# A-Nasiri-M/sap3d_tensorflow

Hardware: AMD Instinct MI355X
Metric: clips/s (16x112x112 fwd+bwd) (higher is better)
Workload: dtype f32

## Files before the change

### include/p3d_hip.h

```cpp
#ifndef P3D_HIP_H
#define P3D_HIP_H
#include <stddef.h>
#include <stdint.h>

#ifdef __cplusplus
extern "C" {
#endif

typedef struct p3d_handle p3d_handle;

enum {
    P3D_STRUCTURE_UNET = 0,
    P3D_STRUCTURE_CONCAT = 1,
    P3D_STRUCTURE_GN_P3D = 2,
    P3D_STRUCTURE_UNETPP_NONSA = 3,
    P3D_STRUCTURE_GN_P3D_DECODER = 4,
    P3D_STRUCTURE_GN_P3D_CONCAT = 5,
    P3D_STRUCTURE_UNETPP_DS = 6
};

typedef struct p3d_config {
    int structure;
    int batch;
    int frames;
// ... 134 lines not shown
                   float b2, float eps, int lr_on_device, float* lr_t);
int p3d_debug_optimizer(int device, int kind, float* p, float* g, float* m, int64_t n, int offset, float lr, float momentum,
                        int use_nesterov, int lr_on_device);
int p3d_debug_optimizer_decay(int device, int kind, float* p, float* g, float* m, int64_t n, int offset, const int64_t* tile_off,
                              const int64_t* tile_len, const float* tile_c, int ntile, float lr, float momentum, int use_nesterov,
                              int lr_on_device, int update, double* term);
int p3d_debug_stat_parts(const int64_t xshape[5], const int64_t wshape[5], const int s[3], int transpose, int* written, int* cap);
int p3d_debug_igemm_groupable(const int64_t xshape[5], const int64_t wshape[5], const int s[3]);
int p3d_op_max_pool3d(int device, const float* x, const int64_t xshape[5], const int ksize[3], const int s[3], float* y);
int p3d_op_max_pool3d_grad(int device, const float* x, const int64_t xshape[5], const int ksize[3], const int s[3],
                           const float* dy, float* dx);
int p3d_op_bias_add_grad(int device, const float* dy, int64_t rows, int channels, float* dbias);
int p3d_debug_conv_launch(int device, int kind, const float* in, int ld_in, int off_in, const int64_t xshape[5], const float* w,
                          const int64_t wshape[5], const int s[3], const float* bias, int accum, int f16, float* out, int ld_out,
                          int off_out, char* kernels, int kernels_cap, int* splits);
int p3d_debug_wgrad_group(int device, int n, const float* const* x, const int* ldx, const int* offx, const int64_t* xs,
                          const float* const* dy, const int* lddy, const int* offdy, const int64_t* ws, const int* s, const int* transpose,
                          float* const* dw, float* const* dbias, int polite, int greedy, char* kernel, int kernel_cap, int* cuts,
                          int* info);
int p3d_debug_max_pool3d(int device, const float* x, int ldx, int offx, const int64_t xshape[5], const int ksize[3], const int s[3],
                         float* y, int ldy, int offy);
int p3d_debug_max_pool3d_grad(int device, const float* x, int ldx, int offx, const int64_t xshape[5], const int ksize[3], const int s[3],
                              const float* dy, int ldy, int offy, int accumulate, float* dx, const char** kernel);
int p3d_debug_bias_add_grad(int device, const float* dy, int64_t rows, int channels, int ld, int off, float* dbias);
int p3d_op_attention_core(int device, int batch, int n_g, int n_f, int ch, const float* g, const float* f, const float* h,
                          float* o, const float* d_o, float* dg, float* df, float* dh);
int p3d_debug_attention_core(int device, int mode, int batch, int n_g, int n_f, int ch, const float* g, const float* f, const float* h,
                             float* o, const float* d_o, float* dg, float* df, float* dh);
int p3d_debug_attention_splits(int batch, int n_g, int n_f, int ch, int splits[4]);
int p3d_debug_softmax_rows(int device, int backward, int64_t rows, int cols, int ld, float* s, float* d, int guard_rows);
// ... 32 lines not shown
```

### sap3d_tensorflow_amd/_lib.py

```python
import ctypes as C
import os

_HERE = os.path.dirname(os.path.abspath(__file__))
LIB_PATH = os.environ.get("P3D_LIB") or os.path.join(_HERE, "libp3dhip.so")

P3D_COMM_ID_BYTES = 128
LOSSES = {"smooth_l1": 0, "bce": 1, "l1": 2}
P3D_LOSS_KLD_CC = 3
MAP_LOSSES = {"kld": (1.0, 0.0), "kld_cc": (1.0, 1.0)}
REGULARIZATION = {"weightdecay": 1, "l2": 2}
OPTIMIZERS = {"adam": 0, "momentum": 1, "sgd": 2}
SLOT_NAMES = {"adam": ("Adam", "Adam_1"), "momentum": ("Momentum",), "sgd": ()}


class P3dConfig(C.Structure):
    _fields_ = [("structure", C.c_int), ("batch", C.c_int), ("frames", C.c_int), ("height", C.c_int),
                ("width", C.c_int), ("base", C.c_int), ("blocks", C.c_int * 3), ("device", C.c_int),
                ("world_size", C.c_int), ("rank", C.c_int)]


class P3dOpTime(C.Structure):
    _fields_ = [("name", C.c_char * 64), ("kernel", C.c_char * 48), ("ms", C.c_double), ("flops", C.c_double),
                ("bytes", C.c_double), ("phase", C.c_int)]

# ... 83 lines not shown
    "p3d_debug_optimizer": (C.c_int, [C.c_int, C.c_int, _fp, _fp, _fp, C.c_int64, C.c_int, C.c_float, C.c_float, C.c_int, C.c_int]),
    "p3d_debug_optimizer_decay": (C.c_int, [C.c_int, C.c_int, _fp, _fp, _fp, C.c_int64, C.c_int, _i64p, _i64p, _fp, C.c_int, C.c_float,
                                            C.c_float, C.c_int, C.c_int, C.c_int, _dp]),
    "p3d_debug_adam": (C.c_int, [C.c_int, _fp, _fp, _fp, _fp, C.c_int64, C.c_int, C.c_float, C.c_int64, C.c_float, C.c_float,
                                 C.c_float, C.c_int, _fp]),
    "p3d_debug_stat_parts": (C.c_int, [_i64p, _i64p, _ip, C.c_int, _ip, _ip]),
    "p3d_debug_igemm_groupable": (C.c_int, [_i64p, _i64p, _ip]),
    "p3d_op_conv3d_backprop_input": (C.c_int, [C.c_int, _fp, _fp, _i64p, _ip, _i64p, _fp]),
    "p3d_op_conv3d_backprop_filter": (C.c_int, [C.c_int, _fp, _i64p, _fp, _i64p, _ip, _fp, _fp]),
    "p3d_op_conv3d_transpose": (C.c_int, [C.c_int, _fp, _i64p, _fp, _i64p, _ip, _fp, _fp]),
    "p3d_op_max_pool3d": (C.c_int, [C.c_int, _fp, _i64p, _ip, _ip, _fp]),
    "p3d_op_max_pool3d_grad": (C.c_int, [C.c_int, _fp, _i64p, _ip, _ip, _fp, _fp]),
    "p3d_op_bias_add_grad": (C.c_int, [C.c_int, _fp, C.c_int64, C.c_int, _fp]),
    "p3d_debug_conv_launch": (C.c_int, [C.c_int, C.c_int, _fp, C.c_int, C.c_int, _i64p, _fp, _i64p, _ip, _fp, C.c_int, C.c_int, _fp,
                                        C.c_int, C.c_int, C.c_char_p, C.c_int, _ip]),
    "p3d_debug_wgrad_group": (C.c_int, [C.c_int, C.c_int, C.POINTER(_fp), _ip, _ip, _i64p, C.POINTER(_fp), _ip, _ip, _i64p, _ip, _ip,
                                        C.POINTER(_fp), C.POINTER(_fp), C.c_int, C.c_int, C.c_char_p, C.c_int, _ip, _ip]),
    "p3d_debug_max_pool3d": (C.c_int, [C.c_int, _fp, C.c_int, C.c_int, _i64p, _ip, _ip, _fp, C.c_int, C.c_int]),
    "p3d_debug_max_pool3d_grad": (C.c_int, [C.c_int, _fp, C.c_int, C.c_int, _i64p, _ip, _ip, _fp, C.c_int, C.c_int, C.c_int, _fp,
                                            C.POINTER(C.c_char_p)]),
    "p3d_debug_bias_add_grad": (C.c_int, [C.c_int, _fp, C.c_int64, C.c_int, C.c_int, C.c_int, _fp]),
    "p3d_op_attention_core": (C.c_int, [C.c_int, C.c_int, C.c_int, C.c_int, C.c_int, _fp, _fp, _fp, _fp, _fp, _fp, _fp, _fp]),
    "p3d_debug_attention_core": (C.c_int, [C.c_int, C.c_int, C.c_int, C.c_int, C.c_int, C.c_int, _fp, _fp, _fp, _fp, _fp, _fp, _fp, _fp]),
    "p3d_debug_attention_splits": (C.c_int, [C.c_int, C.c_int, C.c_int, C.c_int, _ip]),
    "p3d_debug_softmax_rows": (C.c_int, [C.c_int, C.c_int, C.c_int64, C.c_int, C.c_int, _fp, _fp, C.c_int]),
    "p3d_debug_attn_mix": (C.c_int, [C.c_int, C.c_int64, C.c_int, _fp, C.c_int, C.c_int, _fp, C.c_int, C.c_int, C.c_float, C.c_float,
                                     C.c_uint64, C.c_int, _fp, C.c_int, C.c_int, _fp, C.c_int, _fp, _fp, _fp]),
    "p3d_metric_cc": (C.c_int, [C.c_int, _fp, _fp, C.c_int, C.c_int, _dp]),
    "p3d_metric_sim": (C.c_int, [C.c_int, _fp, _fp, C.c_int, C.c_int, _dp]),
    "p3d_metric_nss": (C.c_int, [C.c_int, _fp, _fp, C.c_int, C.c_int, _dp]),
# ... 116 lines not shown
```

### sap3d_tensorflow_amd/csrc/conv_igemm2.hip

```cpp
#if !defined(__gfx950__) && !defined(__gfx942__) && defined(__HIP_DEVICE_COMPILE__)
#error "the K-slice exchange (write-through slab stores + relaxed ticket + one-lane acquire) is written for gfx942 / gfx950 cache semantics"
#endif
#include "p3d_kernels.h"
#include "igemm_epilogue.h"
#include <algorithm>
#include <cstddef>
#include <cstdio>
#include <cstring>
#include <cstdlib>
#include <map>
#include <mutex>
#include <tuple>
#include <vector>

typedef float f32x16 __attribute__((ext_vector_type(16)));
typedef unsigned u32x4 __attribute__((ext_vector_type(4)));

namespace {

constexpr int BK = 32;
#ifndef P3D_RING64
#define P3D_RING64 3
#endif
template <int BM, int BN>
// ... 72 lines not shown
    } else {
#pragma unroll
        for (int i = 0; i < LB; ++i) {
            const int r = (i * 4 + wave) * 8 + a_sub;
            st.bk[i] = 4 * (a_slot ^ ((r >> 1) & 7));
            st.bok[i] = (n0 + r) < p.Nc;
            st.boff[i] = (n0 + r) * p.K + st.bk[i];
        }
    }
    st.t = s_begin / kchunks; st.kc = s_begin - st.t * kchunks; st.issued = 0;
}

template <int LA, bool TWO>
__device__ __forceinline__ void a_set_tap(const IgemmArgs& p, P3dKTap* taps, ALoad<LA, TWO>& st) {
    const P3dTap tap = p3d_ktap(taps, st.t);
#pragma unroll
    for (int i = 0; i < LA; ++i) {
        const int id = (st.dhw[i] >> 20) + tap.dd, ih = ((st.dhw[i] >> 10) & 1023) + tap.dh, iw = (st.dhw[i] & 1023) + tap.dw;
        const bool ok = st.base[i] >= 0 && (unsigned)id < (unsigned)p.Di && (unsigned)ih < (unsigned)p.Hi &&
                        (unsigned)iw < (unsigned)p.Wi;
        const long long row = (long long)st.base[i] + ((long long)id * p.Hi + ih) * p.Wi + iw;
        st.aptr[i] = ok ? p.x + row * p.ldx + st.achunk[i] : nullptr;
        if (TWO) st.aptr2[TWO ? i : 0] = ok ? p.x2 + row * p.ldx2 + st.achunk[i] : nullptr;
    }
}

template <int BM>
__device__ __forceinline__ void issue_a_dma(const IgemmArgs& p, P3dKTap* taps, float* __restrict__ a_dst, ALoad<BM / 32, false>& st, int nsteps,
                                            int kchunks, bool first, int wave, int lane) {
    constexpr int LA = BM / 32;
    const bool live = st.issued < nsteps;
    if (live && (first || st.kc == 0)) a_set_tap(p, taps, st);
    const int k0 = st.kc * BK;
    const float* zp = p.zeros + 4 * (lane & 7);
#pragma unroll
    for (int i = 0; i < LA; ++i) {
        const bool ok = live && st.aptr[i] != nullptr && (k0 + st.achunk[i]) < p.K;
        glds16(ok ? st.aptr[i] + k0 : zp, a_dst + (i * 4 + wave) * 8 * BK);
    }
    ++st.issued;
    if (++st.kc == kchunks) { st.kc = 0; ++st.t; }
}
template <int BN, bool WT>
__device__ __forceinline__ void issue_b_dma(const IgemmArgs& p, P3dKTap* taps, float* __restrict__ b_dst, BLoad<BN / 32>& st, int nsteps, int kchunks,
                                            int wave, int lane) {
    constexpr int LB = BN / 32;
    const bool live = st.issued < nsteps;
    const int k0 = st.kc * BK;
    const float* zp = p.zeros + 4 * (lane & 7);
    const float* wt = st.w + (long long)taps[live ? st.t : 0].widx * p.K * p.Nc;
    if (!WT) {
#pragma unroll
        for (int i = 0; i < LB; ++i) {
            const bool ok = live && st.bok[i] && (k0 + st.bk[i]) < p.K;
            glds16(ok ? wt + (long long)k0 * p.Nc + st.boff[i] : zp, b_dst + (i * 4 + wave) * 256);
        }
    } else {
#pragma unroll
        for (int i = 0; i < LB; ++i) {
            const bool ok = live && st.bok[i] && (k0 + st.bk[i]) < p.K;
            glds16(ok ? wt + k0 + st.boff[i] : zp, b_dst + (i * 4 + wave) * 8 * BK);
        }
    }
    ++st.issued;
    if (++st.kc == kchunks) { st.kc = 0; ++st.t; }
// ... 709 lines not shown
    if (pl.splits > 1 && pl.splits > a.ntaps * ((a.K + BK - 1) / BK)) return hipErrorInvalidValue;
    if (a.at_mode != P3D_AT_NONE) {
        const long long kp = (long long)((a.K + BK - 1) / BK) * BK;
        if (kp * 4 > MAX_TABLE_FLOATS) return hipErrorInvalidValue;
        if ((a.at_mode == P3D_AT_RELU2 || a.at_mode == P3D_AT_GRAD) && (!a.x2 || (a.ldx2 & 3))) return hipErrorInvalidValue;
    }
    if (a.at_mode == P3D_AT_RELU1 || a.at_mode == P3D_AT_RELU2) {
        if (a.f1.part && (a.f1.nparts < 1 || a.f1.nparts > P3D_FOLD_MAX)) return hipErrorInvalidValue;
        if (a.at_mode == P3D_AT_RELU2 && a.f2.part && (a.f2.nparts < 1 || a.f2.nparts > P3D_FOLD_MAX)) return hipErrorInvalidValue;
    }
    if (a.at_mode == P3D_AT_GRAD && a.gf.part && (a.gf.nparts < 1 || a.gf.nparts > P3D_FOLD_MAX)) return hipErrorInvalidValue;
    if (a.ngate < 0 || a.ngate > 2) return hipErrorInvalidValue;
    for (int q = 0; q < a.ngate; ++q)
        if (!a.gate[q].y || !a.gate[q].out || !a.gate[q].part || (a.gate[q].ldy & 3) || (a.gate[q].ldo & 3)) return hipErrorInvalidValue;
    if (a.ngate && a.statpart) return hipErrorInvalidValue;
    if (pl.stream_blocks > 0) return p3d_launch_pw_stream(a, s);
    if (p3d_igemm2_tail_split(a, pl)) return p3d_launch_igemm2_group(&a, 1, pl, s);
    if (pl.bm == 128 && pl.bn == 128) return launch_t<128, 128>(a, pl, s);
    if (pl.bm == 128 && pl.bn == 64) return launch_t<128, 64>(a, pl, s);
    return launch_t<64, 64>(a, pl, s);
}

bool p3d_igemm2_groupable(const IgemmArgs* v, int n, const P3dIgemmPlan& pl) {
    if (n < 2 || n > P3D_IGEMM_CLASSES) return false;
    for (int i = 0; i < n; ++i) {
        const IgemmArgs& a = v[i];
        if (a.at_mode != P3D_AT_NONE || a.ngate || a.x != v[0].x || a.wT != v[0].wT || a.K != v[0].K || a.Nc != v[0].Nc || a.N != v[0].N ||
            a.f16 != v[0].f16 || a.accum != v[0].accum || a.ldx != v[0].ldx || a.ldy != v[0].ldy || a.Di != v[0].Di || a.Hi != v[0].Hi ||
            a.Wi != v[0].Wi || a.Do != v[0].Do || a.Ho != v[0].Ho || a.Wo != v[0].Wo || a.isd != v[0].isd || a.ish != v[0].ish ||
            a.isw != v[0].isw || a.osd != v[0].osd || a.osh != v[0].osh || a.osw != v[0].osw)
            return false;
        const P3dIgemmPlan q = p3d_igemm2_plan(a, 1);
        if (q.bm != pl.bm || q.bn != pl.bn) return false;
        if (q.stream_blocks > 0) return false;
    }
    return true;
}

namespace {
template <int BM, int BN>
hipError_t launch_group_t(IgemmGroupArgs& g, const long long* tiles, hipStream_t s) {
    long long blocks = 0, slabs = 0, counters = 0;
// ... 102 lines not shown
```

### sap3d_tensorflow_amd/csrc/net.hip

```cpp
#include "../../include/p3d_hip.h"
#include "p3d_kernels.h"

#include <rccl/rccl.h>

#include <algorithm>
#include <atomic>
#include <cmath>
#include <cstdio>
#include <cstring>
#include <deque>
#include <functional>
#include <map>
#include <memory>
#include <mutex>
#include <stdexcept>
#include <string>
#include <vector>

namespace {

thread_local std::string g_err;

struct RuntimeEnv { bool debug_sync = false, graph = false, no_side_stream = false; };
const RuntimeEnv& runtime_env() {
// ... 215 lines not shown
void igemm_work(const IgemmArgs& a, double& flops, double& bytes) {
    const double M = (double)a.N * a.Gd * a.Gh * a.Gw;
    const double side = (double)a.N * a.Di * a.Hi * a.Wi;
    const double gathered = std::min(M * std::max(a.ntaps, 1), side);
    flops = 2.0 * M * a.ntaps * (double)a.K * a.Nc;
    bytes = 4.0 * (gathered * a.K + M * a.Nc * (1 + a.accum) + (double)a.ntaps * a.K * a.Nc);
}

void launch_igemm(const Ctx& c, const IgemmArgs& a0, int allow_split = 0) {
    IgemmArgs a = a0;
    double fl, by;
    igemm_work(a, fl, by);
    a.zeros = g_zero_page;
    const P3dIgemmPlan pl = p3d_igemm2_plan(a, allow_split);
    const char* name = pl.name;
    if (a.f16) name = pl.bm == 128 ? (pl.bn == 128 ? "igemm2_kernel<128,128,f16>" : "igemm2_kernel<128,64,f16>") : "igemm2_kernel<64,64,f16>";
    else if (a.at_mode || a.ngate) {
        static const char* const tiles[3] = {"64,64", "128,64", "128,128"};
        static const char* const ats[4] = {"", ",relu1", ",relu2", ",bngrad"};
        static std::map<int, std::string> names;
        const int key = (pl.bm == 128 ? (pl.bn == 128 ? 2 : 1) : 0) * 8 + a.at_mode * 2 + (a.ngate ? 1 : 0);
        std::string& nm = names[key];
        if (nm.empty()) nm = std::string("igemm2_kernel<") + tiles[key / 8] + ats[a.at_mode] + (a.ngate ? ",gate" : "") + ">";
        name = nm.c_str();
    }
    launch(c, name, fl, by, [&]() { return p3d_launch_igemm2(a, pl, c.s); });
}

void zero_strided(const Ctx& c, float* p, int ld, int64_t rows, int C);

struct StatSink { float* part = nullptr; int cap = 0; int* nparts = nullptr; };
// ... 437 lines not shown
                            a.taps[t].dd = (int16_t)((pd + g.pad[0] - kd) / g.s[0]);
                            a.taps[t].dh = (int16_t)((ph + g.pad[1] - kh) / g.s[1]);
                            a.taps[t].dw = (int16_t)((pw + g.pad[2] - kw) / g.s[2]);
                            a.taps[t].widx = (int16_t)((kd * g.k[1] + kh) * g.k[2] + kw);
                            ++t;
                        }
                    }
                }
                a.ntaps = t;
                if (t == 0 && !include_empty) continue;
                v.push_back(a);
            }
    return v;
}

void stem_filter_gradient(const Ctx& c, const StemGeo& sg, const float* x4, const float* dy, int ldy, float* dw4, float* dw, float* dbias,
                          bool greedy, float* onepass_part = nullptr, const BnBwdArgs* through_bn = nullptr) {
    const ConvGeo& g = sg.g;
    const int N = sg.N, Wp = sg.Wp, Cout = sg.Cout, KH = sg.KH, K4 = sg.K4;
    if (onepass_part && !dbias && sg.part_floats) {
        StemWgradArgs a;
        memset(&a, 0, sizeof(a));
        a.x4 = x4; a.Wp = Wp; a.Hi = g.I[1]; a.nimg = N * g.I[0]; a.Ho = g.O[1]; a.Wo = g.O[2]; a.pad_h = g.pad[1];
        a.dy = dy; a.lddy = ldy; a.part = onepass_part; a.dw = dw;
        if (through_bn) {
            const BnBwdArgs& b = *through_bn;
            a.fused = 1; a.dy = b.dz; a.lddy = b.lddz; a.y = b.y1; a.ldy = b.ld1;
            a.scale = b.scale1; a.shift = b.shift1; a.mean = b.mean1; a.invstd = b.invstd1; a.gamma = b.gamma1; a.coef = b.coef1; a.batch = b.batch1;
        }
        const double rows = (double)a.nimg * a.Ho * a.Wo;
// ... 416 lines not shown
        if (fold) { f.part = statpart_arena + bn->gpart_off; f.nparts = bn->gnparts; }
        f.publish = (fold && publish) ? 1 : 0;
        return f;
    }
    BnGate bn_gate(const FuseSrc& s) {
        BnGate g;
        memset(&g, 0, sizeof(g));
        g.y = s.y->p; g.ldy = s.y->ld;
        g.scale = s.bn->scale; g.shift = s.bn->shift; g.mean = s.bn->mean; g.invstd = s.bn->invstd;
        g.out = s.y->g; g.ldo = s.y->ld;
        g.part = statpart_arena + s.bn->gpart_off;
        return g;
    }

    std::vector<IgemmArgs> sib_pending;

#include "net_ops.inc"
#include "net_gn.inc"
#include "net_graphs.inc"
#include "net_plan.inc"
#include "net_sched.inc"
};

#include "net_abi.inc"
```

### sap3d_tensorflow_amd/csrc/net_abi.inc

```
#define API_BEGIN try {
#define API_END                                        \
    }                                                  \
    catch (const std::exception& e) {                  \
        g_err = e.what();                              \
        return -1;                                     \
    }                                                  \
    return 0;

extern "C" {

const char* p3d_last_error(void) { return g_err.c_str(); }

void p3d_default_config(p3d_config* c) {
    memset(c, 0, sizeof(*c));
    c->structure = P3D_STRUCTURE_UNET;
    c->batch = 2; c->frames = 16; c->height = 112; c->width = 112; c->base = 64;
    c->blocks[0] = 3; c->blocks[1] = 8; c->blocks[2] = 36;
    c->device = 0; c->world_size = 1; c->rank = 0;
}

static void refuse_two_hip_runtimes() {
    FILE* f = fopen("/proc/self/maps", "r");
    if (!f) return;
    std::vector<std::string> seen;
// ... 550 lines not shown
    Act* a = it->second.in; Act* b = it->second.out;
    if (in_count != a->rows() * a->C || out_count != b->rows() * b->C) throw P3dError("block tensor size mismatch");
    if (!a->g || !b->g) throw P3dError("this bottleneck's input or output carries no gradient");
    HIPCHECK(hipSetDevice(h->cfg.device));
    HIPCHECK(hipMemcpy2DAsync(a->p, (size_t)a->ld * 4, in, (size_t)a->C * 4, (size_t)a->C * 4, (size_t)a->rows(), hipMemcpyHostToDevice, h->stream));
    Ctx c; c.training = true; c.s = h->stream; c.fuse = false;
    h->sib_pending.clear();
    h->last_forward_fused = false;
    if (h->stats_count) HIPCHECK(hipMemsetAsync(h->stats_arena, 0, (size_t)h->stats_count * sizeof(double), c.s));
    for (size_t i = it->second.op0; i < it->second.op1; ++i) h->ops[i].fwd(c);
    h->zeroed_early = false;
    h->zero_backward_arenas(c.s, true);
    c.z0 = h->zb; c.z1 = h->zb + h->zb_bytes;
    HIPCHECK(hipMemcpy2DAsync(b->g, (size_t)b->ld * 4, dout, (size_t)b->C * 4, (size_t)b->C * 4, (size_t)b->rows(), hipMemcpyHostToDevice, c.s));
    h->wq.clear(); h->wq_flushes = 0; h->parked_flops = 0;
    for (size_t i = it->second.op1; i-- > it->second.op0;) {
        c.bwd_op = h->ops[i].name.c_str();
        h->ops[i].bwd(c);
    }
    h->flush_wgrads(c);
    HIPCHECK(hipMemcpy2DAsync(din, (size_t)a->C * 4, a->g, (size_t)a->ld * 4, (size_t)a->C * 4, (size_t)a->rows(), hipMemcpyDeviceToHost, c.s));
    HIPCHECK(hipStreamSynchronize(c.s));
    API_END
}

int p3d_profile_step(p3d_handle* h, float dropout_rate, uint64_t seed, p3d_op_time* out, int cap) {
    if (!h) { g_err = "null handle"; return -1; }
    try {
        HIPCHECK(hipSetDevice(h->cfg.device));
        Prof prof;
// ... 881 lines not shown
    if (v.size() == 1 && p3d_igemm2_tail_split(v[0], p3d_igemm2_plan(v[0], 1))) names += "(tail)";
    put_string(names, kernels, kernels_cap);
    if (splits) {
        splits[0] = 1 << 30; splits[1] = 0;
        for (const IgemmArgs& a : v) {
            const P3dIgemmPlan pl = p3d_igemm2_plan(a, 1);
            const int sp = pl.stream_blocks > 0 || pl.splits < 1 ? 1 : pl.splits;
            splits[0] = std::min(splits[0], sp); splits[1] = std::max(splits[1], sp);
        }
        if (v.empty()) splits[0] = splits[1] = 0;
    }
    dout.get(out, rout * ld_out);
    API_END
}

int p3d_debug_wgrad_group(int device, int n, const float* const* x, const int* ldx, const int* offx, const int64_t* xs,
                          const float* const* dy, const int* lddy, const int* offdy, const int64_t* ws, const int* s, const int* transpose,
                          float* const* dw, float* const* dbias, int polite, int greedy, char* kernel, int kernel_cap, int* cuts,
                          int* info) {
    API_BEGIN
    HIPCHECK(hipSetDevice(device));
    if (!x || !ldx || !offx || !xs || !dy || !lddy || !offdy || !ws || !s || !transpose || !dw || !dbias || !cuts || !info)
        throw P3dError("null argument");
    if (n < 1 || n > P3D_WGRAD_GROUP) throw P3dError("wgrad_group: 1 to " + std::to_string(P3D_WGRAD_GROUP) + " problems");
    struct Bufs { std::unique_ptr<DevBuf> x, dy, dw, db; int64_t nw; int nb; };
    std::vector<Bufs> bufs((size_t)n);
    std::vector<WgradArgs> probs;
    ensure_zero_page();
    double fl = 0, by = 0;
    for (int i = 0; i < n; ++i) {
// ... 614 lines not shown
```

### sap3d_tensorflow_amd/csrc/net_ops.inc

```
    Act* conv(const std::string& opname, Act* x, Param* w, Param* bias, const int k[3], const int s[3], int Cout, BN* bn,
              const std::string& out_name, bool stem = false, bool bn_has_dropout = false, int sibling = 0,
              const ConvFuse* fuse = nullptr) {
        const ConvGeo g = make_geo(x->D, x->H, x->W, k, s);
        Act* y = new_act(out_name, x->N, g.O[0], g.O[1], g.O[2], Cout);
        if (bn && stats_target(bn, y->rows(), Cout, bn_has_dropout)) reserve_stat_parts(bn, y->rows());
        const ConvFuse cf = fuse ? *fuse : ConvFuse();
        if (cf.out_bn) { if (cf.out_bn != bn) throw P3dError("fused output BatchNorm must be the conv's own"); make_fusable(bn, y->rows()); }
        if (cf.ngate && (s[0] != 1 || s[1] != 1 || s[2] != 1)) throw P3dError("gated input gradients need a stride-1 conv");
        char* xflag = x->g ? consume(x) : nullptr;
        const int Cin = x->C;
        const int ntap = k[0] * k[1] * k[2];
        Op op;
        op.name = opname; op.kind = stem ? "conv_stem" : (ntap == 1 ? "conv_1x1x1" : "conv_kxkxk");
        op.flops = 2.0 * y->rows() * ntap * Cin * Cout;
        op.bytes = 4.0 * (x->rows() * (double)Cin + y->rows() * (double)Cout + (double)ntap * Cin * Cout);
        op.bflops = op.flops * (x->g ? 2 : 1);
        op.bbytes = op.bytes * (x->g ? 2 : 1);
        op.owns = {w}; if (bias) op.owns.push_back(bias);
        if (cf.out_bn) { op.owns.push_back(cf.out_bn->gamma); op.owns.push_back(cf.out_bn->beta); }
        hipEvent_t fork_ev = new_fork_event();
        if (stem) {
            if (k[0] != 1 || Cin != 3 || bias) throw P3dError("stem path is for [1,kh,kw,3,C] kernels without bias");
            const StemGeo sg = stem_geo(g, x->N, Cout);
            float* x4 = dalloc<float>(sg.x4_floats);
// ... 59 lines not shown
            if (fin) {
                wa.xt = cf.at == P3D_AT_RELU2 ? 2 : 1;
                wa.xs1 = cf.src[0].bn->scale; wa.xt1 = cf.src[0].bn->shift;
                if (wa.xt == 2) { wa.x2 = cf.src[1].y->p; wa.ldx2 = cf.src[1].y->ld; wa.xs2 = cf.src[1].bn->scale; wa.xt2 = cf.src[1].bn->shift; }
            }
            return wa;
        };
        op.bwd = [=](const Ctx& c) {
            if (!(c.fuse_bwd && cf.any())) {
                queue_wgrad(c, wgrad_args(c.fuse && cf.at != 0));
                if (xflag) {
                    const int accum = *xflag;
                    auto v = igemm_conv_input_side(g, x->N, y->g, y->ld, Cout, x->g, x->ld, Cin, w->p, nullptr, accum,
                                                   !accum);
                    if (f16()) for (auto& a : v) a.f16 = 1;
                    run_igemm_group(c, v, accum != 0, nullptr);
                }
                return;
            }
            WgradArgs wa = wgrad_args(cf.at != 0);
            if (cf.out_bn) { wa.dyt = 1; wa.dy2 = y->p; wa.ldy2 = y->ld; wa.dcoef = cf.out_bn->coef; }
            if (!xflag) throw P3dError("a conv with a fused BatchNorm needs an input gradient launch (it publishes the coefficients)");
            if (cf.out_bn && !c.dry) {
                grad_finalized[cf.out_bn] = false;
                if (cf.out_bn->gnparts > FOLD_MAX) {
                    const BnGradFold gf = bn_grad_fold(cf.out_bn, y->rows(), true);
                    launch(c, "bn_grad_finalize_kernel", 0, 64.0 * cf.out_bn->C, [&]() { return p3d_bn_grad_finalize(gf, c.s); });
                    grad_finalized[cf.out_bn] = true;
                }
            }
// ... 218 lines not shown
```

### sap3d_tensorflow_amd/csrc/net_sched.inc

```
    void debug_sync(const char* dir, const Op& op, const Ctx& c) {
        if (!runtime_env().debug_sync) return;
        fprintf(stderr, "[p3d] %s %s (%s) ...", dir, op.name.c_str(), op.kind.c_str());
        fflush(stderr);
        HIPCHECK(hipStreamSynchronize(c.s));
        fprintf(stderr, " ok\n");
        fflush(stderr);
    }
    void run_forward(const Ctx& c) {
        sib_pending.clear();
        if (stats_count) HIPCHECK(fill_async(stats_arena, 0, (size_t)stats_count * sizeof(double), c.s, "statistics"));
        if (zf_bytes) HIPCHECK(fill_async(zf, 0, zf_bytes, c.s, "forward-arena"));
        Ctx cz = c; cz.z0 = zf; cz.z1 = zf + zf_bytes;
        cz.fuse = fuse_bn && !c.per_sample && !c.dry;
        last_forward_fused = cz.fuse;
        if (!c.dry) pred_ready = true;
        const bool no_side_f = runtime_env().no_side_stream;
        cz.side = (c.prof || no_side_f || c.dry) ? nullptr : side_stream;
        const Ctx& c2 = cz;
        for (auto& op : ops) {
            if (c.prof) c.prof->cur_op = op.name;
            op.fwd(c2);
            debug_sync("fwd", op, c);
        }
    }
// ... 40 lines not shown
        c.fuse_bwd = c.fuse && fuse_bn_bwd;
        bool adam_done = false;
        const bool no_side = runtime_env().no_side_stream;
        c.side = (c.prof || no_side) ? nullptr : side_stream;
        if (zeroed_early) {
            zeroed_early = false;
            HIPCHECK(ev_wait(c.s, ev_zeroed));
            if (zb_bytes) HIPCHECK(fill_async(zb, 0, zb_bytes, c.s, "backward-arena"));
        } else {
            zero_backward_arenas(c.s, true);
        }
        for (auto& a : acts) if (a.stem_link) a.stem_link->pending = false;
        int64_t hi = n_train;
        size_t own_pos = own_sorted.size();
        wq.clear(); wq_flushes = 0;
        std::vector<std::pair<hipEvent_t, std::function<void(const Ctx&)>>> parked;
        bool early_adam = false, early_comm = false;
        static const bool no_defer = p3d_tune_env("P3D_DEFER_SIDE") && atoi(p3d_tune_env("P3D_DEFER_SIDE")) == 0;
        const bool defer_on = c.side && !no_defer && defer_release_op > 0 && defer_budget > 0;
        parked_flops = 0;
        auto release_parked = [&]() {
            c.defer = nullptr;
            bool first = true;
            for (auto& job : parked) {
                if (first || !c.side) on_side_stream(c, job.first, job.second);
                else { Ctx sc = c; sc.s = c.side; job.second(sc); }
                first = false;
            }
            parked.clear();
        };
// ... 304 lines not shown
```

### sap3d_tensorflow_amd/csrc/p3d_kernels.h

```cpp
#pragma once
#include <hip/hip_runtime.h>
#include <stdint.h>

#define P3D_MAX_TAPS 27
#ifndef P3D_WGRAD_GROUP
#define P3D_WGRAD_GROUP 6
#endif
#define P3D_STAT_REPLICAS 16
#define P3D_FOLD_MAX 32

#include <stdlib.h>
inline const char* p3d_tune_env(const char* name) {
#if defined(P3D_TUNING)
    return getenv(name);
#else
    (void)name;
    return nullptr;
#endif
}

struct P3dFastDiv { unsigned mul; int shift; };
inline P3dFastDiv p3d_fastdiv(unsigned d) {
    P3dFastDiv f{0u, 0};
    if (d <= 1) return f;
// ... 30 lines not shown
    else if constexpr (LINES >= 6)
        asm volatile(P3D_WL4(0x0, 0x40, 0x80, 0xc0) P3D_WL(0x100) P3D_WL(0x140) "s_waitcnt lgkmcnt(0)" : "=&s"(t) : "s"(ka) : "memory");
    else if constexpr (LINES >= 4)
        asm volatile(P3D_WL4(0x0, 0x40, 0x80, 0xc0) "s_waitcnt lgkmcnt(0)" : "=&s"(t) : "s"(ka) : "memory");
    else if constexpr (LINES >= 2)
        asm volatile(P3D_WL(0x0) P3D_WL(0x40) "s_waitcnt lgkmcnt(0)" : "=&s"(t) : "s"(ka) : "memory");
}
template <class Args>
__device__ __forceinline__ void p3d_warm_kernargs() { p3d_warm_kernarg_lines<(int)((sizeof(Args) + 63) / 64)>(); }
#endif

struct P3dTap {
    int16_t dd, dh, dw;
    int16_t widx;
};

struct BnFold {
    const float* gamma; const float* beta;
    const float* part; int nparts;
    int C;
    float* scale; float* shift; float* mean; float* invstd;
    float* moving_mean; float* moving_var;
    double inv_m;
    float eps; int publish; int update_moving;
};
struct BnGradFold {
    const float* gamma; const float* mean; const float* invstd;
    const float* part; int nparts;
    int C;
    float* coef;
// ... 21 lines not shown
    int ldy;
    int Nc;
    int osd, osh, osw, ood, ooh, oow;
    const float* w;
    int wT;
    const float* bias;
    float* statpart;
    int stat_base;
    int accum;
    const float* zeros;
    float* slab; unsigned* cnt; int nsplit;
    int f16;
    int xcd_min_tiles;
    int at_mode;
    const float* x2; int ldx2;
    BnFold f1, f2;
    BnGradFold gf;
    int ngate, raw_store;
    BnGate gate[2];
    int ntaps;
    P3dTap taps[P3D_MAX_TAPS];
};

#define P3D_IGEMM_CLASSES 8
struct IgemmClass {
    int Gd, Gh, Gw;
    P3dFastDiv fGd, fGh, fGw;
    int ood, ooh, oow;
    int stat_base;
    int ntaps;
// ... 385 lines not shown
```

### sap3d_tensorflow_amd/ops.py

```python
import ctypes as C

import numpy as np

from ._lib import LOSSES, OPTIMIZERS, check, fptr, lib


def _f32(a):
    return np.ascontiguousarray(a, dtype=np.float32)


def _shape5(s):
    return (C.c_int64 * 5)(*[int(v) for v in s])


def _i3(s):
    return (C.c_int * 3)(*[int(v) for v in s])


def _same_out(size, s):
    return -(-size // s)


def _strides3(strides):
    strides = list(strides)
# ... 185 lines not shown
    l_in, l_out = (c if v is None else int(v) for v, c in zip(ld, (ci, co)))
    o_in, o_out = (int(v) for v in offset)
    xin = _embed(x.reshape(-1, ci), l_in, o_in, pad)
    rows_out = int(np.prod(oshape[:4]))
    pr = np.broadcast_to(np.asarray(prior, np.float32), oshape).reshape(rows_out, co)
    out = _embed(pr, l_out, o_out, pad)
    b = _f32(bias) if bias is not None else None
    names = C.create_string_buffer(16384)
    splits = (C.c_int * 2)()
    check(lib().p3d_debug_conv_launch(device, kd, fptr(xin), l_in, o_in, _shape5(xshape), fptr(w), _shape5(w.shape), _i3(s), fptr(b),
                                      1 if accum else 0, 1 if f16 else 0, fptr(out), l_out, o_out, names, len(names), splits))
    conv_launch.last_splits = (splits[0], splits[1])
    return out[:, o_out:o_out + co].reshape(oshape).copy(), _outside(out, co, o_out), names.value.decode()


def wgrad_group(problems, polite=False, greedy=False, pad=np.nan, device=0):
    n = len(problems)
    xs, dys, dws, dbs, keep = [], [], [], [], []
    ldx, offx, lddy, offdy, tr = [], [], [], [], []
    xsh, wsh, st = [], [], []
    for pr in problems:
        x, dy = _f32(pr["x"]), _f32(pr["dy"])
        fs = tuple(int(v) for v in pr["filter_sizes"])
        l = pr.get("ld", (None, None))
        o = pr.get("offset", (0, 0))
        lx, ly = (c if v is None else int(v) for v, c in zip(l, (x.shape[4], dy.shape[4])))
        xs.append(_embed(x.reshape(-1, x.shape[4]), lx, int(o[0]), pad))
        dys.append(_embed(dy.reshape(-1, dy.shape[4]), ly, int(o[1]), pad))
        dws.append(np.zeros(fs, np.float32) if pr.get("dw") is None else _f32(np.asarray(pr["dw"]).reshape(fs)).copy())
        dbs.append(None if pr.get("dbias") is None else _f32(np.asarray(pr["dbias"]).reshape(fs[3] if pr.get("transpose") else fs[4])).copy())
# ... 287 lines not shown
```

Baseline: 531.8.

## Fuse sibling conv input gradients into one K-concatenated implicit GEMM launch

```diff
diff --git a/include/p3d_hip.h b/include/p3d_hip.h
--- a/include/p3d_hip.h
+++ b/include/p3d_hip.h
@@ -172,6 +172,9 @@
 int p3d_debug_conv_launch(int device, int kind, const float* in, int ld_in, int off_in, const int64_t xshape[5], const float* w,
                           const int64_t wshape[5], const int s[3], const float* bias, int accum, int f16, float* out, int ld_out,
                           int off_out, char* kernels, int kernels_cap, int* splits);
+int p3d_debug_conv_launch_cat(int device, const int64_t xshape[5], const float* dy1, int ld1, int off1, const float* w1,
+                              const int64_t wshape1[5], const float* dy2, int ld2, int off2, const float* w2, const int64_t wshape2[5],
+                              int accum, float* out, int ld_out, int off_out, char* kernels, int kernels_cap, int* splits);
 int p3d_debug_wgrad_group(int device, int n, const float* const* x, const int* ldx, const int* offx, const int64_t* xs,
                           const float* const* dy, const int* lddy, const int* offdy, const int64_t* ws, const int* s, const int* transpose,
                           float* const* dw, float* const* dbias, int polite, int greedy, char* kernel, int kernel_cap, int* cuts,
diff --git a/sap3d_tensorflow_amd/_lib.py b/sap3d_tensorflow_amd/_lib.py
--- a/sap3d_tensorflow_amd/_lib.py
+++ b/sap3d_tensorflow_amd/_lib.py
@@ -121,6 +121,8 @@
     "p3d_op_bias_add_grad": (C.c_int, [C.c_int, _fp, C.c_int64, C.c_int, _fp]),
     "p3d_debug_conv_launch": (C.c_int, [C.c_int, C.c_int, _fp, C.c_int, C.c_int, _i64p, _fp, _i64p, _ip, _fp, C.c_int, C.c_int, _fp,
                                         C.c_int, C.c_int, C.c_char_p, C.c_int, _ip]),
+    "p3d_debug_conv_launch_cat": (C.c_int, [C.c_int, _i64p, _fp, C.c_int, C.c_int, _fp, _i64p, _fp, C.c_int, C.c_int, _fp, _i64p, C.c_int,
+                                            _fp, C.c_int, C.c_int, C.c_char_p, C.c_int, _ip]),
     "p3d_debug_wgrad_group": (C.c_int, [C.c_int, C.c_int, C.POINTER(_fp), _ip, _ip, _i64p, C.POINTER(_fp), _ip, _ip, _i64p, _ip, _ip,
                                         C.POINTER(_fp), C.POINTER(_fp), C.c_int, C.c_int, C.c_char_p, C.c_int, _ip, _ip]),
     "p3d_debug_max_pool3d": (C.c_int, [C.c_int, _fp, C.c_int, C.c_int, _i64p, _ip, _ip, _fp, C.c_int, C.c_int]),
diff --git a/sap3d_tensorflow_amd/csrc/conv_igemm2.hip b/sap3d_tensorflow_amd/csrc/conv_igemm2.hip
--- a/sap3d_tensorflow_amd/csrc/conv_igemm2.hip
+++ b/sap3d_tensorflow_amd/csrc/conv_igemm2.hip
@@ -110,13 +110,16 @@
 template <int LA, bool TWO>
 __device__ __forceinline__ void a_set_tap(const IgemmArgs& p, P3dKTap* taps, ALoad<LA, TWO>& st) {
     const P3dTap tap = p3d_ktap(taps, st.t);
+    const bool src2 = !TWO && (tap.widx & P3D_TAP_SRC2);
+    const float* const xb = src2 ? p.x2 : p.x;
+    const int ldb = src2 ? p.ldx2 : p.ldx;
 #pragma unroll
     for (int i = 0; i < LA; ++i) {
         const int id = (st.dhw[i] >> 20) + tap.dd, ih = ((st.dhw[i] >> 10) & 1023) + tap.dh, iw = (st.dhw[i] & 1023) + tap.dw;
         const bool ok = st.base[i] >= 0 && (unsigned)id < (unsigned)p.Di && (unsigned)ih < (unsigned)p.Hi &&
                         (unsigned)iw < (unsigned)p.Wi;
         const long long row = (long long)st.base[i] + ((long long)id * p.Hi + ih) * p.Wi + iw;
-        st.aptr[i] = ok ? p.x + row * p.ldx + st.achunk[i] : nullptr;
+        st.aptr[i] = ok ? xb + row * ldb + st.achunk[i] : nullptr;
         if (TWO) st.aptr2[TWO ? i : 0] = ok ? p.x2 + row * p.ldx2 + st.achunk[i] : nullptr;
     }
 }
@@ -144,7 +147,8 @@
     const bool live = st.issued < nsteps;
     const int k0 = st.kc * BK;
     const float* zp = p.zeros + 4 * (lane & 7);
-    const float* wt = st.w + (long long)taps[live ? st.t : 0].widx * p.K * p.Nc;
+    const int widx = taps[live ? st.t : 0].widx;
+    const float* wt = ((widx & P3D_TAP_SRC2) ? p.w2 : st.w) + (long long)P3D_TAP_SLAB(widx) * p.K * p.Nc;
     if (!WT) {
 #pragma unroll
         for (int i = 0; i < LB; ++i) {
@@ -884,6 +888,11 @@
     for (int q = 0; q < a.ngate; ++q)
         if (!a.gate[q].y || !a.gate[q].out || !a.gate[q].part || (a.gate[q].ldy & 3) || (a.gate[q].ldo & 3)) return hipErrorInvalidValue;
     if (a.ngate && a.statpart) return hipErrorInvalidValue;
+    for (int t = 0; t < a.ntaps; ++t) {
+        if (a.taps[t].widx < 0 || (a.taps[t].widx & ~(P3D_TAP_SRC2 | 0xff))) return hipErrorInvalidValue;
+        if ((a.taps[t].widx & P3D_TAP_SRC2) && (!a.x2 || !a.w2 || (a.ldx2 & 3) || a.at_mode != P3D_AT_NONE || pl.stream_blocks > 0))
+            return hipErrorInvalidValue;
+    }
     if (pl.stream_blocks > 0) return p3d_launch_pw_stream(a, s);
     if (p3d_igemm2_tail_split(a, pl)) return p3d_launch_igemm2_group(&a, 1, pl, s);
     if (pl.bm == 128 && pl.bn == 128) return launch_t<128, 128>(a, pl, s);
@@ -895,7 +904,7 @@
     if (n < 2 || n > P3D_IGEMM_CLASSES) return false;
     for (int i = 0; i < n; ++i) {
         const IgemmArgs& a = v[i];
-        if (a.at_mode != P3D_AT_NONE || a.ngate || a.x != v[0].x || a.wT != v[0].wT || a.K != v[0].K || a.Nc != v[0].Nc || a.N != v[0].N ||
+        if (a.at_mode != P3D_AT_NONE || a.ngate || a.w2 || a.x != v[0].x || a.wT != v[0].wT || a.K != v[0].K || a.Nc != v[0].Nc || a.N != v[0].N ||
             a.f16 != v[0].f16 || a.accum != v[0].accum || a.ldx != v[0].ldx || a.ldy != v[0].ldy || a.Di != v[0].Di || a.Hi != v[0].Hi ||
             a.Wi != v[0].Wi || a.Do != v[0].Do || a.Ho != v[0].Ho || a.Wo != v[0].Wo || a.isd != v[0].isd || a.ish != v[0].ish ||
             a.isw != v[0].isw || a.osd != v[0].osd || a.osh != v[0].osh || a.osw != v[0].osw)
diff --git a/sap3d_tensorflow_amd/csrc/net.hip b/sap3d_tensorflow_amd/csrc/net.hip
--- a/sap3d_tensorflow_amd/csrc/net.hip
+++ b/sap3d_tensorflow_amd/csrc/net.hip
@@ -253,7 +253,8 @@
     a.zeros = g_zero_page;
     const P3dIgemmPlan pl = p3d_igemm2_plan(a, allow_split);
     const char* name = pl.name;
-    if (a.f16) name = pl.bm == 128 ? (pl.bn == 128 ? "igemm2_kernel<128,128,f16>" : "igemm2_kernel<128,64,f16>") : "igemm2_kernel<64,64,f16>";
+    if (a.w2) name = pl.bm == 128 ? (pl.bn == 128 ? "igemm2_kernel<128,128>(k-cat)" : "igemm2_kernel<128,64>(k-cat)") : "igemm2_kernel<64,64>(k-cat)";
+    else if (a.f16) name = pl.bm == 128 ? (pl.bn == 128 ? "igemm2_kernel<128,128,f16>" : "igemm2_kernel<128,64,f16>") : "igemm2_kernel<64,64,f16>";
     else if (a.at_mode || a.ngate) {
         static const char* const tiles[3] = {"64,64", "128,64", "128,128"};
         static const char* const ats[4] = {"", ",relu1", ",relu2", ",bngrad"};
@@ -721,6 +722,23 @@
     return v;
 }
 
+constexpr int CONCAT_MIN_K = 64;
+bool igemm_concat_input_gradients(IgemmArgs& a, const IgemmArgs& b) {
+    if (a.K < CONCAT_MIN_K || a.ntaps + b.ntaps > P3D_MAX_TAPS || a.ntaps < 1 || b.ntaps < 1) return false;
+    if (a.at_mode != P3D_AT_NONE || b.at_mode != P3D_AT_NONE || a.ngate || b.ngate || a.f16 || b.f16 || a.bias || b.bias || a.w2 || b.w2) return false;
+    if (a.y != b.y || a.ldy != b.ldy || a.Nc != b.Nc || a.K != b.K || a.wT != b.wT || a.N != b.N || a.Di != b.Di || a.Hi != b.Hi || a.Wi != b.Wi ||
+        a.Gd != b.Gd || a.Gh != b.Gh || a.Gw != b.Gw || a.isd != b.isd || a.ish != b.ish || a.isw != b.isw || a.Do != b.Do || a.Ho != b.Ho ||
+        a.Wo != b.Wo || a.osd != b.osd || a.osh != b.osh || a.osw != b.osw || a.ood != b.ood || a.ooh != b.ooh || a.oow != b.oow)
+        return false;
+    a.x2 = b.x; a.ldx2 = b.ldx; a.w2 = b.w;
+    for (int t = 0; t < b.ntaps; ++t) {
+        P3dTap tap = b.taps[t];
+        tap.widx = (int16_t)(tap.widx | P3D_TAP_SRC2);
+        a.taps[a.ntaps++] = tap;
+    }
+    return true;
+}
+
 void stem_filter_gradient(const Ctx& c, const StemGeo& sg, const float* x4, const float* dy, int ldy, float* dw4, float* dw, float* dbias,
                           bool greedy, float* onepass_part = nullptr, const BnBwdArgs* through_bn = nullptr) {
     const ConvGeo& g = sg.g;
@@ -1167,6 +1185,7 @@
     }
 
     std::vector<IgemmArgs> sib_pending;
+    std::vector<IgemmArgs> sib_bwd_pending;
 
 #include "net_ops.inc"
 #include "net_gn.inc"
diff --git a/sap3d_tensorflow_amd/csrc/net_abi.inc b/sap3d_tensorflow_amd/csrc/net_abi.inc
--- a/sap3d_tensorflow_amd/csrc/net_abi.inc
+++ b/sap3d_tensorflow_amd/csrc/net_abi.inc
@@ -588,6 +588,7 @@
     c.z0 = h->zb; c.z1 = h->zb + h->zb_bytes;
     HIPCHECK(hipMemcpy2DAsync(b->g, (size_t)b->ld * 4, dout, (size_t)b->C * 4, (size_t)b->C * 4, (size_t)b->rows(), hipMemcpyHostToDevice, c.s));
     h->wq.clear(); h->wq_flushes = 0; h->parked_flops = 0;
+    h->sib_bwd_pending.clear();
     for (size_t i = it->second.op1; i-- > it->second.op0;) {
         c.bwd_op = h->ops[i].name.c_str();
         h->ops[i].bwd(c);
@@ -1499,6 +1500,38 @@
     API_END
 }
 
+int p3d_debug_conv_launch_cat(int device, const int64_t xs[5], const float* dy1, int ld1, int off1, const float* w1, const int64_t ws1[5],
+                              const float* dy2, int ld2, int off2, const float* w2, const int64_t ws2[5], int accum, float* out, int ld_out,
+                              int off_out, char* kernels, int kernels_cap, int* splits) {
+    API_BEGIN
+    HIPCHECK(hipSetDevice(device));
+    if (!xs || !dy1 || !w1 || !ws1 || !dy2 || !w2 || !ws2 || !out) throw P3dError("null argument");
+    const int one[3] = {1, 1, 1};
+    const ConvProblem p1 = conv_problem(xs, ws1, one, 0), p2 = conv_problem(xs, ws2, one, 0);
+    if (p1.stem || p2.stem) throw P3dError("conv_launch_cat: the stem shape has its own entry points");
+    if (ws1[3] != p1.Cin || ws2[3] != p2.Cin) throw P3dError("filter Cin mismatch");
+    check_slice("conv_launch_cat (first gradient)", ld1, off1, p1.Cout);
+    check_slice("conv_launch_cat (second gradient)", ld2, off2, p2.Cout);
+    check_slice("conv_launch_cat (output side)", ld_out, off_out, p1.Cin);
+    DevBuf d1(p1.rows * ld1, dy1), d2(p2.rows * ld2, dy2), dw1(prod5(ws1), w1), dw2(prod5(ws2), w2), dout(p1.rows_in * ld_out, out);
+    ensure_zero_page();
+    std::vector<IgemmArgs> v = p1.input_gradient(d1.p + off1, dw1.p, dout.p + off_out, ld1, ld_out, accum ? 1 : 0);
+    const std::vector<IgemmArgs> u = p2.input_gradient(d2.p + off2, dw2.p, dout.p + off_out, ld2, ld_out, 1);
+    if (v.size() != 1 || u.size() != 1 || !igemm_concat_input_gradients(v[0], u[0]))
+        throw P3dError("conv_launch_cat: the two input gradients do not go out as one K-concatenated launch");
+    Ctx c;
+    std::string names;
+    traced_kernels([&]() { run_igemm_group(c, v, accum != 0, nullptr); }, names);
+    if (p3d_igemm2_tail_split(v[0], p3d_igemm2_plan(v[0], 1))) names += "(tail)";
+    put_string(names, kernels, kernels_cap);
+    if (splits) {
+        const P3dIgemmPlan pl = p3d_igemm2_plan(v[0], 1);
+        splits[0] = splits[1] = pl.stream_blocks > 0 || pl.splits < 1 ? 1 : pl.splits;
+    }
+    dout.get(out, p1.rows_in * ld_out);
+    API_END
+}
+
 int p3d_debug_wgrad_group(int device, int n, const float* const* x, const int* ldx, const int* offx, const int64_t* xs,
                           const float* const* dy, const int* lddy, const int* offdy, const int64_t* ws, const int* s, const int* transpose,
                           float* const* dw, float* const* dbias, int polite, int greedy, char* kernel, int kernel_cap, int* cuts,
diff --git a/sap3d_tensorflow_amd/csrc/net_ops.inc b/sap3d_tensorflow_amd/csrc/net_ops.inc
--- a/sap3d_tensorflow_amd/csrc/net_ops.inc
+++ b/sap3d_tensorflow_amd/csrc/net_ops.inc
@@ -97,6 +97,23 @@
                     auto v = igemm_conv_input_side(g, x->N, y->g, y->ld, Cout, x->g, x->ld, Cin, w->p, nullptr, accum,
                                                    !accum);
                     if (f16()) for (auto& a : v) a.f16 = 1;
+                    if (sibling == 2 && !c.dry && v.size() == 1 && v[0].K >= CONCAT_MIN_K) {
+                        if (!sib_bwd_pending.empty()) throw P3dError("sibling conv " + opname + ": an earlier pair never sent its input gradient");
+                        v[0].accum = accum;
+                        sib_bwd_pending.push_back(v[0]);
+                        return;
+                    }
+                    if (sibling == 1 && !sib_bwd_pending.empty()) {
+                        std::vector<IgemmArgs> first;
+                        first.swap(sib_bwd_pending);
+                        IgemmArgs m = first[0];
+                        if (v.size() == 1 && accum && igemm_concat_input_gradients(m, v[0])) {
+                            first[0] = m;
+                            run_igemm_group(c, first, m.accum != 0, nullptr);
+                            return;
+                        }
+                        run_igemm_group(c, first, first[0].accum != 0, nullptr);
+                    }
                     run_igemm_group(c, v, accum != 0, nullptr);
                 }
                 return;
diff --git a/sap3d_tensorflow_amd/csrc/net_sched.inc b/sap3d_tensorflow_amd/csrc/net_sched.inc
--- a/sap3d_tensorflow_amd/csrc/net_sched.inc
+++ b/sap3d_tensorflow_amd/csrc/net_sched.inc
@@ -78,6 +78,7 @@
         int64_t hi = n_train;
         size_t own_pos = own_sorted.size();
         wq.clear(); wq_flushes = 0;
+        sib_bwd_pending.clear();
         std::vector<std::pair<hipEvent_t, std::function<void(const Ctx&)>>> parked;
         bool early_adam = false, early_comm = false;
         static const bool no_defer = p3d_tune_env("P3D_DEFER_SIDE") && atoi(p3d_tune_env("P3D_DEFER_SIDE")) == 0;
diff --git a/sap3d_tensorflow_amd/csrc/p3d_kernels.h b/sap3d_tensorflow_amd/csrc/p3d_kernels.h
--- a/sap3d_tensorflow_amd/csrc/p3d_kernels.h
+++ b/sap3d_tensorflow_amd/csrc/p3d_kernels.h
@@ -68,6 +68,8 @@
     int16_t dd, dh, dw;
     int16_t widx;
 };
+#define P3D_TAP_SRC2 0x100
+#define P3D_TAP_SLAB(widx) ((widx) & 0xff)
 
 struct BnFold {
     const float* gamma; const float* beta;
@@ -119,6 +121,7 @@
     int xcd_min_tiles;
     int at_mode;
     const float* x2; int ldx2;
+    const float* w2;
     BnFold f1, f2;
     BnGradFold gf;
     int ngate, raw_store;
diff --git a/sap3d_tensorflow_amd/ops.py b/sap3d_tensorflow_amd/ops.py
--- a/sap3d_tensorflow_amd/ops.py
+++ b/sap3d_tensorflow_amd/ops.py
@@ -223,6 +223,26 @@
     return out[:, o_out:o_out + co].reshape(oshape).copy(), _outside(out, co, o_out), names.value.decode()
 
 
+def conv_launch_cat(dy1, filter1, dy2, filter2, input_sizes, accum=False, ld=(None, None, None), offset=(0, 0, 0), pad=np.nan,
+                    prior=np.nan, device=0):
+    g1, g2, w1, w2 = _f32(dy1), _f32(dy2), _f32(filter1), _f32(filter2)
+    xshape = tuple(int(v) for v in input_sizes)
+    c1, c2, co = g1.shape[4], g2.shape[4], xshape[4]
+    l1, l2, l_out = (c if v is None else int(v) for v, c in zip(ld, (c1, c2, co)))
+    o1, o2, o_out = (int(v) for v in offset)
+    in1, in2 = _embed(g1.reshape(-1, c1), l1, o1, pad), _embed(g2.reshape(-1, c2), l2, o2, pad)
+    rows_out = int(np.prod(xshape[:4]))
+    pr = np.broadcast_to(np.asarray(prior, np.float32), xshape).reshape(rows_out, co)
+    out = _embed(pr, l_out, o_out, pad)
+    names = C.create_string_buffer(16384)
+    splits = (C.c_int * 2)()
+    check(lib().p3d_debug_conv_launch_cat(device, _shape5(xshape), fptr(in1), l1, o1, fptr(w1), _shape5(w1.shape), fptr(in2), l2, o2,
+                                          fptr(w2), _shape5(w2.shape), 1 if accum else 0, fptr(out), l_out, o_out, names, len(names),
+                                          splits))
+    conv_launch_cat.last_splits = (splits[0], splits[1])
+    return out[:, o_out:o_out + co].reshape(xshape).copy(), _outside(out, co, o_out), names.value.decode()
+
+
 def wgrad_group(problems, polite=False, greedy=False, pad=np.nan, device=0):
     n = len(problems)
     xs, dys, dws, dbs, keep = [], [], [], [], []
```

Result: no change. 535.4 (median of 6 runs) (+0.7%).
